# rampasek/GraphGPS

Hardware: NVIDIA H100
Metric: graphs/sec GPSLayer fwd+bwd (higher is better)
Workload: dtype f32

## Files before the change

graphgps_b200/_lib.py:

```python
from __future__ import annotations

import ctypes as C
import os

import torch

_HERE = os.path.dirname(os.path.abspath(__file__))
LIB_PATH = os.path.join(_HERE, "libgps_b200.so")

GPS_OK, GPS_ERR_ARG, GPS_ERR_UNSUPPORTED, GPS_ERR_CUDA = 0, -1, -2, -3
LOCAL = {"None": 0, "CustomGatedGCN": 1, "GINE": 2, "GCN": 3}
GLOBAL = {"None": 0, "Transformer": 1, "Performer": 2}
ACT = {"relu": 0, "gelu": 1}
PRECISION = {"fp32": 0, "bf16": 1}
NORM = {"batch": 0, "none": 1}

_fp = C.c_void_p


class GpsGraph(C.Structure):
    _fields_ = [("N", C.c_int64), ("E", C.c_int64), ("B", C.c_int64),
                ("dst_ptr", _fp), ("dst_src", _fp), ("dst_eid", _fp),
                ("src_ptr", _fp), ("src_dst", _fp), ("src_eid", _fp), ("graph_ptr", _fp)]

# ... 23 lines not shown
        ("x", _fp), ("edge_attr", _fp), ("x_out", _fp), ("edge_out", _fp),
        ("gcn_A", GpsLinear), ("gcn_B", GpsLinear), ("gcn_C", GpsLinear), ("gcn_D", GpsLinear),
        ("gcn_E", GpsLinear),
        ("bn_node_x", GpsBatchNorm), ("bn_edge_e", GpsBatchNorm),
        ("gine_lin0", GpsLinear), ("gine_lin1", GpsLinear),
        ("attn_in", GpsLinear), ("attn_out", GpsLinear),
        ("perf_q", GpsLinear), ("perf_k", GpsLinear), ("perf_v", GpsLinear),
        ("perf_proj", _fp), ("perf_features", C.c_int64), ("perf_dim_head", C.c_int64),
        ("norm1_local", GpsBatchNorm), ("norm1_attn", GpsBatchNorm), ("norm2", GpsBatchNorm),
        ("ff1", GpsLinear), ("ff2", GpsLinear),
        ("grad_x_out", _fp), ("grad_edge_out", _fp), ("grad_x", _fp), ("grad_edge_attr", _fp),
        ("saved", _fp), ("saved_bytes", C.c_int64),
        ("workspace", _fp), ("workspace_bytes", C.c_int64),
        ("offset_dev", _fp),
        ("gcn_conv", GpsLinear),
        ("ev_grads_early", _fp),
        ("x_planes_in", GpsPlanes), ("e_planes_in", GpsPlanes), ("x_planes_out", GpsPlanes), ("e_planes_out", GpsPlanes),
        ("wplanes", _fp), ("wplanes_bytes", C.c_int64), ("wplanes_valid", C.c_int32), ("reserved2", C.c_int32),
        ("ev_grads_mid", _fp), ("ev_grads_done", _fp),
        ("pe", _fp), ("pe_dim", C.c_int64), ("grad_pe", _fp), ("pe_mlp0", GpsLinear), ("pe_mlp1", GpsLinear),
    ]


class GpsLayerPlan(C.Structure):
    _fields_ = [("saved_bytes", C.c_int64), ("fwd_workspace_bytes", C.c_int64),
                ("bwd_workspace_bytes", C.c_int64), ("fwd_launches", C.c_int64),
                ("bwd_launches", C.c_int64), ("wplanes_bytes", C.c_int64)]


_i64, _i32, _f32, _u64 = C.c_int64, C.c_int32, C.c_float, C.c_uint64
SYMBOLS = {
    "gps_last_error": (C.c_char_p, []),
    "gps_abi_version": (C.c_int, []),
    "gps_build_arch": (C.c_char_p, []),
    "gps_graph_bytes": (_i64, [_i64, _i64, _i64]),
    "gps_graph_build": (C.c_int, [_fp, _fp, _i64, _i64, _i64, _fp, _i64, C.POINTER(GpsGraph), _fp]),
    "gps_layer_plan": (C.c_int, [C.POINTER(GpsLayerArgs), C.POINTER(GpsLayerPlan)]),
    "gps_layer_forward": (C.c_int, [C.POINTER(GpsLayerArgs), _fp]),
    "gps_layer_backward": (C.c_int, [C.POINTER(GpsLayerArgs), _fp]),
    "gps_linear_forward": (C.c_int, [_fp, _i64, _fp, _i64, _fp, _fp, _i64, _i64, _i64, _i64, _i32, _i32, _fp]),
    "gps_gemm": (C.c_int, [_fp, _i64, _i32, _fp, _i64, _i32, _fp, _i64, _i64, _i64, _i64, _i32, _i32, _i32, _fp]),
    "gps_gatedgcn_aggregate_forward": (C.c_int, [C.POINTER(GpsGraph), _i64, _fp, _fp, _fp, _fp, _i64, _fp, _fp,
                                                 _fp, _fp, _fp]),
    "gps_gine_aggregate_forward": (C.c_int, [C.POINTER(GpsGraph), _i64, _fp, _fp, _f32, _fp, _fp]),
    "gps_gatedgcn_aggregate_forward_gated": (C.c_int, [C.POINTER(GpsGraph), _i64, _fp, _fp, _fp, _fp, _i64, _fp, _fp,
                                                       _fp, _fp, _fp, _fp]),
    "gps_gatedgcn_aggregate_backward": (C.c_int, [C.POINTER(GpsGraph), _i64, _fp, _fp, _i64, _fp, _fp, _i64, _fp, _fp,
                                                  _fp, C.POINTER(GpsPlanes), C.POINTER(GpsPlanes), _fp]),
    "gps_eslap_forward": (C.c_int, [C.POINTER(GpsGraph), _fp, _i64, _i64, _i32, _fp, _fp, _fp, _fp, _fp, _fp, _fp]),
    "gps_eslap_workspace_bytes": (_i64, [_i64, _i64]),
    "gps_eslap_backward": (C.c_int, [C.POINTER(GpsGraph), _fp, _i64, _i64, _i32, _fp, _fp, _fp, _i64, _fp, _fp, _fp,
                                     _fp, _fp, _fp, _fp, _i64, _fp, _fp, _fp, _fp, _fp, _i32, _fp]),
    "gps_gine_aggregate_backward": (C.c_int, [C.POINTER(GpsGraph), _i64, _fp, _fp, _fp, _f32, _fp, _fp, _fp, _fp]),
    "gps_gcn_aggregate_forward": (C.c_int, [C.POINTER(GpsGraph), _i64, _fp, _i64, _fp, _fp, _fp, _fp, _f32, _u64, _u64,
                                            _fp, _fp]),
    "gps_gcn_aggregate_backward": (C.c_int, [C.POINTER(GpsGraph), _i64, _fp, _fp, _fp, _i64, C.POINTER(GpsPlanes), _fp]),
    "gps_attention_forward": (C.c_int, [C.POINTER(GpsGraph), _i64, _i64, _fp, _fp, _fp, _i64, _fp, _i64, _fp,
                                        _f32, _u64, _u64, _fp]),
    "gps_attention_backward": (C.c_int, [C.POINTER(GpsGraph), _i64, _i64, _fp, _fp, _fp, _i64, _fp, _fp, _i64,
                                         _fp, _fp, _fp, _fp, _fp, _i64, _f32, _u64, _u64, _fp]),
    "gps_attention_forward_tc": (C.c_int, [C.POINTER(GpsGraph), _i64, _i64, _fp, _fp, _i64, _fp, _i64, _fp, _f32, _u64, _u64,
                                           _i32, _fp]),
    "gps_dropout_mask": (C.c_int, [_fp, _i64, _i64, _f32, _u64, _u64, _i32, _fp]),
    "gps_to_planes": (C.c_int, [_fp, _i64, _i64, _i64, _fp, _fp, _i64, _fp]),
    "gps_gemm_planes": (C.c_int, [_fp, _fp, _i64, _i32, _fp, _fp, _i64, _i32, _fp, _i64, _fp, _fp, _i64, _i64, _i64, _i64,
                                  _i32, _i32, _fp, _fp]),
    "gps_fallback_count": (C.c_ulonglong, []),
    "gps_launch_count": (C.c_ulonglong, []),
    "gps_debug_set": (None, [C.c_int]),
    "gps_debug_tma": (None, [C.c_int, _fp]),
    "gps_debug_attn": (None, [_fp]),
}

_lib = None


def load():
    global _lib
    if _lib is not None:
        return _lib
    if not os.path.exists(LIB_PATH):
        raise RuntimeError(
            f"{LIB_PATH} not found: build it with `python -m graphgps_b200.build` "
            "(nvcc, sm_90a). graphgps_b200 has no CPU/eager fallback.")
    lib = C.CDLL(LIB_PATH)
    for name, (res, args) in SYMBOLS.items():
        fn = getattr(lib, name)
        fn.restype = res
        fn.argtypes = args
    if lib.gps_abi_version() != 3:
        raise RuntimeError("libgps_b200.so ABI version mismatch")
    _lib = lib
    return lib
# ... 20 lines not shown
```

graphgps_b200/csrc/gemm.cuh:

```cuda
#pragma once
#include <cuda.h>

#include "common.cuh"

namespace gps {

struct GemmParams {
  int M = 0, N = 0, K = 0;
  const float* A = nullptr; int lda = 0; int ta = 0;
  const float* B = nullptr; int ldb = 0; int tb = 0;
  float* C = nullptr; int ldc = 0;
  const float* bias = nullptr;
  float* C_pre = nullptr; int ldpre = 0;
  int act = -1;
  const float* mask_src = nullptr; int ldmask = 0; int mask_act = -1;
  int mask_is_post = 0;
  float p_drop = 0.f; uint64_t seed = 0, offset = 0; int site = 0;
  const unsigned long long* offset_dev = nullptr;
  float p_drop2 = 0.f; int site2 = 0;
  const float* R1 = nullptr; int ldr1 = 0;
  const float* R2 = nullptr; int ldr2 = 0;
  double* stats = nullptr;
  int splitk = 1;
  float* colsum_a = nullptr;
  int precision = GPS_PREC_FP32;
  Planes Ap, Bp, Cp;
  int cp_hd = 0, cp_hd_pad = 0, cp_col0 = 0;
  struct BnRed { const float* z = nullptr; int ldz = 0; const float* mean = nullptr; const float* invstd = nullptr; double* sums = nullptr; };
  BnRed bnred[2];
};

struct ToPlanesItem { const float* src; int64_t ld; int rows; int cols; Planes dst; };
int to_planes(const ToPlanesItem* items, int n, cudaStream_t stream);
int gemm_tma(const GemmParams& p, cudaStream_t stream);
int make_tensor_map(const __nv_bfloat16* hi, const __nv_bfloat16* lo, int planes, int64_t rows, int64_t cols, int64_t ld,
                    int box_rows, CUtensorMap* out);
void gemm_tma_set_force_bn(int bn);
void gemm_tma_set_trace(unsigned long long* buf);

int gemm_simt(const GemmParams& p, cudaStream_t stream);
int gemm_tc(const GemmParams& p, cudaStream_t stream);
void gemm_tc_set_debug(int v);
int gemm(const GemmParams& p, cudaStream_t stream);

}
```

graphgps_b200/csrc/gemm_tma.cu:

```cuda
#include <cooperative_groups.h>
#include <cuda.h>
#include <cuda_bf16.h>

#include <mutex>
#include <unordered_map>

#include "gemm.cuh"
#include "tc_ptx.cuh"

namespace gps {

namespace {

using namespace tc;
namespace cgrp = cooperative_groups;

constexpr int BM = 128;
constexpr int BK = 64;
constexpr int kEpiWarps = 8;
constexpr int kTmaWarp = 8;
constexpr int kThreads = 288;
constexpr int kATile = BM * BK * 2;
constexpr int kBlock = 64 * BK * 2;
constexpr int kMaxSplits = 8;

struct TmaArgs {
  GemmParams p;
  int BN, nb_blocks, stages, kb_per_split, planes;
  int debug;
  unsigned long long* trace;
};

__device__ __forceinline__ unsigned long long gtimer() {
  unsigned long long t;
  asm volatile("mov.u64 %0, %globaltimer;" : "=l"(t));
  return t;
}
#define GPS_TRACE(slot)                                                                         \
  do {                                                                                          \
    if (a.trace && cta_lin < 256) a.trace[cta_lin * 16 + (slot)] = gtimer();                    \
  } while (0)

template <bool A_MN, bool B_MN, int BN_T, bool SPLIT>
__global__ void __launch_bounds__(kThreads, BN_T == 64 ? 2 : 1)
k_gemm_tma(const __grid_constant__ CUtensorMap tmA, const __grid_constant__ CUtensorMap tmB, const TmaArgs a) {
  extern __shared__ __align__(1024) uint8_t smem_raw[];
  const GemmParams& p = a.p;
  uint8_t* smem = reinterpret_cast<uint8_t*>((reinterpret_cast<uintptr_t>(smem_raw) + 1023) & ~(uintptr_t)1023);
  const int planes = a.planes;
  const int b_tile = B_MN ? a.nb_blocks * kBlock : BN_T * 128;
  const int stage_bytes = planes * (kATile + b_tile);
  const int S = a.stages;
  uint64_t* bars = reinterpret_cast<uint64_t*>(smem + (size_t)S * stage_bytes);
  float* red = reinterpret_cast<float*>(bars + 2 * S + 2);
  float* ctot = red + 16 * 16 * 8;
  const int nsplit = (int)gridDim.z;

  const int tid = threadIdx.x, warp = tid >> 5, lane = tid & 31;
  const int m0 = blockIdx.y * BM, n0 = blockIdx.x * a.BN;
  const int nkb_total = (p.K + BK - 1) / BK;
  const int kb_begin = blockIdx.z * a.kb_per_split;
  const int kb_end = min(nkb_total, kb_begin + a.kb_per_split);
  const int nkb = kb_end - kb_begin;
  const bool do_colsum = A_MN && p.colsum_a != nullptr && blockIdx.x == 0;
  const int cta_lin = (blockIdx.z * gridDim.y + blockIdx.y) * gridDim.x + blockIdx.x;

  if (tid == 0) {
    GPS_TRACE(0);
    if (a.trace && cta_lin < 256) {
      unsigned smid;
      asm volatile("mov.u32 %0, %smid;" : "=r"(smid));
      a.trace[cta_lin * 16 + 8] = smid;
    }
    for (int s = 0; s < S; ++s) {
      mbar_init(smem_u32(&bars[s]), 1);
      mbar_init(smem_u32(&bars[S + s]), kEpiWarps);
    }
    fence_barrier_init();
  }
  if (warp == kTmaWarp && lane == 0) {
    tma_prefetch_desc(&tmA);
    tma_prefetch_desc(&tmB);
  }
  __syncthreads();
  if (tid == 0) GPS_TRACE(1);

  if (warp == kTmaWarp) {
// ... 9 lines not shown
        const uint32_t full = smem_u32(&bars[s]);
        mbar_arrive_expect_tx(full, tx);
        const int k0 = (kb_begin + i) * BK;
        const uint32_t sa = smem_u32(smem + (size_t)s * stage_bytes);
        const uint32_t sb = sa + planes * kATile;
        for (int pl = 0; pl < planes; ++pl) {
          if (!A_MN) {
            tma_tile_3d(sa + pl * kATile, &tmA, k0, m0, pl, full);
          } else {
            for (int b = 0; b < a_blocks; ++b) tma_tile_3d(sa + pl * kATile + b * kBlock, &tmA, m0 + 64 * b, k0, pl, full);
          }
          if (!B_MN) {
            tma_tile_3d(sb + pl * b_tile, &tmB, k0, n0, pl, full);
          } else {
            for (int b = 0; b < b_blocks; ++b) tma_tile_3d(sb + pl * b_tile + b * kBlock, &tmB, n0 + 64 * b, k0, pl, full);
          }
        }
        if (i == 0) GPS_TRACE(2);
      }
      GPS_TRACE(9);
    }
    __syncwarp();
    if (nsplit > 1) {
      cgrp::this_cluster().sync();
      cgrp::this_cluster().sync();
    }
  } else {
    const int wg = warp >> 2;
    float acc[BN_T / 2];
#pragma unroll
    for (int e = 0; e < BN_T / 2; ++e) acc[e] = 0.f;
    float csum[8];
#pragma unroll
    for (int e = 0; e < 8; ++e) csum[e] = 0.f;
    const int cm = tid & 15, kq = tid >> 4;
    constexpr uint32_t a_lbo = A_MN ? kBlock : 16, b_lbo = B_MN ? kBlock : 16;
    constexpr uint32_t a_kstep = A_MN ? 2048 : 32, b_kstep = B_MN ? 2048 : 32;
    for (int i = 0; i < nkb; ++i) {
      const int s = i % S;
      if (lane == 0) mbar_wait(smem_u32(&bars[s]), (uint32_t)(i / S) & 1u);
      __syncwarp();
      if (i == 0 && tid == 0) GPS_TRACE(3);
      if (i == nkb - 1 && tid == 0) GPS_TRACE(10);
      const uint8_t* st = smem + (size_t)s * stage_bytes;
      const uint32_t sa_hi = smem_u32(st) + (uint32_t)wg * 8192u;
      const uint32_t sb_hi = smem_u32(st) + planes * kATile;
      const uint32_t sa_lo = sa_hi + kATile;
      const uint32_t sb_lo = sb_hi + b_tile;
// ... 70 lines not shown
      cgrp::cluster_group cluster = cgrp::this_cluster();
      cluster.sync();
      const int c4n = a.BN >> 2;
      for (int idx = tid; idx < (hi - lo) * c4n; idx += kEpiWarps * 32) {
        const int r = lo + idx / c4n, c = (idx % c4n) * 4;
        float4 sum = f4zero();
        for (int k = 0; k < nsplit; ++k)
          sum = f4add(sum, *reinterpret_cast<const float4*>(cluster.map_shared_rank(stage, k) + r * sld + c));
        *reinterpret_cast<float4*>(stage + r * sld + c) = sum;
      }
      if (do_colsum && blockIdx.z == 0 && tid < 128 && m0 + tid < p.M) {
        float tot = 0.f;
        for (int k = 0; k < nsplit; ++k) tot += cluster.map_shared_rank(ctot, k)[tid];
        atomicAdd(&p.colsum_a[m0 + tid], tot);
      }
      cluster.sync();
    }
    const int G = a.BN >> 2;
    const int rpp = kEpiWarps * 32 / G;
    const int rip = tid / G, cg = tid - rip * G;
    const int col = n0 + cg * 4;
    const bool col_ok = rip < rpp && col < p.N;
    const int rows_here = min(BM, p.M - m0);
    const bool colstats = p.stats || p.bnred[0].sums || p.bnred[1].sums;
    if (col_ok) {
      const int nrows = rip < rows_here ? (rows_here - rip + rpp - 1) / rpp : 0;
      const int64_t row0 = m0 + rip;
      float* sp = stage + rip * sld + cg * 4;
      const int s_st = rpp * sld;
      float* cp = p.C ? p.C + row0 * p.ldc + col : nullptr;
      const int64_t c_st = (int64_t)rpp * p.ldc;
      const float* r1 = p.R1 ? p.R1 + row0 * p.ldr1 + col : nullptr;
      const int64_t r1_st = (int64_t)rpp * p.ldr1;
      const float* r2 = p.R2 ? p.R2 + row0 * p.ldr2 + col : nullptr;
      const int64_t r2_st = (int64_t)rpp * p.ldr2;
      if (p.splitk > 1) {
        for (int r = lo + rip; r < min(hi, rows_here); r += rpp) {
          const int64_t row = m0 + r;
          float4 w = *reinterpret_cast<const float4*>(stage + r * sld + cg * 4);
          if (p.R1) w = f4add(w, ld4(p.R1 + row * p.ldr1 + col));
          if (p.R2) w = f4add(w, ld4(p.R2 + row * p.ldr2 + col));
          atomicAdd(reinterpret_cast<float4*>(p.C + row * p.ldc + col), w);
        }
      } else {
        const bool fast = !p.C_pre && !(p.mask_src && !p.mask_is_post) && p.p_drop == 0.f && p.p_drop2 == 0.f &&
                          (p.act < 0 || p.act == GPS_ACT_RELU);
        const float4 bb = p.bias ? ld4(p.bias + col) : f4zero();
        const float* mk = p.mask_src ? p.mask_src + row0 * p.ldmask + col : nullptr;
        const int64_t mk_st = (int64_t)rpp * p.ldmask;
        int pcol = col, npad = 0;
        if (p.cp_hd > 0) {
          const int cl = col - (p.cp_col0), hq = cl / p.cp_hd, cw = cl - hq * p.cp_hd;
          pcol = hq * p.cp_hd_pad + cw;
          npad = (cw + 4 == p.cp_hd) ? p.cp_hd_pad - p.cp_hd : 0;
        }
        __nv_bfloat16* ph = p.Cp.hi ? p.Cp.hi + row0 * p.Cp.ld + pcol : nullptr;
        __nv_bfloat16* pl = p.Cp.lo ? p.Cp.lo + row0 * p.Cp.ld + pcol : nullptr;
        const int64_t p_st = (int64_t)rpp * p.Cp.ld;
        const bool relu = p.act == GPS_ACT_RELU;
        if (fast) {
// ... 67 lines not shown
            if (r1) w = f4add(w, ld4(r1 + k * r1_st));
            if (r2) w = f4add(w, ld4(r2 + k * r2_st));
            if (cp) st4(cp + k * c_st, w);
            if (ph) {
              planes_store4(p.Cp, row, pcol, w);
              for (int z = 0; z < npad; z += 4) planes_store4(p.Cp, row, pcol + 4 + z, f4zero());
            }
            if (colstats) *reinterpret_cast<float4*>(sp + k * s_st) = w;
          }
        }
      }
    }
    if (colstats) {
      asm volatile("bar.sync 1, 256;" ::: "memory");
      for (int t = tid; t < 16 * G; t += kEpiWarps * 32) {
        const int y = t / G, g = t - y * G, c = n0 + g * 4;
        if (c >= p.N) continue;
        const GemmParams::BnRed& b0 = p.bnred[0];
        const GemmParams::BnRed& b1 = p.bnred[1];
        float4 bm0 = f4zero(), bi0 = f4zero(), bm1 = f4zero(), bi1 = f4zero();
        if (b0.sums) { bm0 = f4scale(ld4(b0.mean + c), -1.f); bi0 = ld4(b0.invstd + c); }
        if (b1.sums) { bm1 = f4scale(ld4(b1.mean + c), -1.f); bi1 = ld4(b1.invstd + c); }
        float4 s1 = f4zero(), s2 = f4zero(), q0 = f4zero(), q1 = f4zero();
        for (int r = y; r < rows_here; r += 16) {
          const float4 w = *reinterpret_cast<const float4*>(stage + r * sld + g * 4);
          const int64_t row = m0 + r;
          s1 = f4add(s1, w);
          s2 = f4fma(w, w, s2);
          if (b0.sums) q0 = f4fma(w, f4mul(f4add(ld4(b0.z + row * b0.ldz + c), bm0), bi0), q0);
          if (b1.sums) q1 = f4fma(w, f4mul(f4add(ld4(b1.z + row * b1.ldz + c), bm1), bi1), q1);
        }
        float* o = stage + y * sld + g * 4;
        *reinterpret_cast<float4*>(o) = s1;
        *reinterpret_cast<float4*>(o + 16 * sld) = s2;
        *reinterpret_cast<float4*>(o + 32 * sld) = q0;
        *reinterpret_cast<float4*>(o + 48 * sld) = q1;
      }
      asm volatile("bar.sync 1, 256;" ::: "memory");
      if (tid < G && n0 + tid * 4 < p.N) {
        float4 t[4] = {f4zero(), f4zero(), f4zero(), f4zero()};
        for (int y = 0; y < 16; ++y)
#pragma unroll
          for (int k = 0; k < 4; ++k) t[k] = f4add(t[k], *reinterpret_cast<const float4*>(stage + (y + 16 * k) * sld + tid * 4));
        const int c0 = n0 + tid * 4;
        auto add4 = [&](double* dst, float4 v) {
          atomic_add_f64(dst + 0, (double)v.x); atomic_add_f64(dst + 1, (double)v.y);
          atomic_add_f64(dst + 2, (double)v.z); atomic_add_f64(dst + 3, (double)v.w);
        };
        if (p.stats) {
          add4(p.stats + c0, t[0]);
          add4(p.stats + (int64_t)p.N + c0, t[1]);
        }
        if (p.bnred[0].sums) {
          add4(p.bnred[0].sums + c0, t[0]);
          add4(p.bnred[0].sums + (int64_t)p.N + c0, t[2]);
        }
        if (p.bnred[1].sums) {
          add4(p.bnred[1].sums + c0, t[0]);
          add4(p.bnred[1].sums + (int64_t)p.N + c0, t[3]);
        }
      }
    }
  }

  if (tid == 0) GPS_TRACE(6);
  if (a.trace) {
// ... 95 lines not shown
    cudaLaunchConfig_t cfg = {};
    cfg.gridDim = grid;
    cfg.blockDim = dim3(kThreads);
    cfg.dynamicSmemBytes = smem;
    cfg.stream = stream;
    cudaLaunchAttribute attr[1];
    attr[0].id = cudaLaunchAttributeClusterDimension;
    attr[0].val.clusterDim.x = 1;
    attr[0].val.clusterDim.y = 1;
    attr[0].val.clusterDim.z = grid.z;
    cfg.attrs = attr;
    cfg.numAttrs = 1;
    GPS_CUDA(cudaLaunchKernelEx(&cfg, k_gemm_tma<A_MN, B_MN, BN_T, SPLIT>, tA, tB, a));
  }
  GPS_LAUNCH_CHECK();
  return GPS_OK;
}
template <bool A_MN, bool B_MN, int BN_T>
int launch(const CUtensorMap& tA, const CUtensorMap& tB, const TmaArgs& a, dim3 grid, size_t smem, cudaStream_t stream) {
  return a.planes == 2 ? launch1<A_MN, B_MN, BN_T, true>(tA, tB, a, grid, smem, stream)
                       : launch1<A_MN, B_MN, BN_T, false>(tA, tB, a, grid, smem, stream);
}

int g_tma_force_bn = 0;
unsigned long long* g_tma_trace = nullptr;
int g_tma_debug = 0;

}

void gemm_tma_set_force_bn(int bn) { g_tma_force_bn = bn & 0xFFFF; g_tma_debug = bn >> 16; }
void gemm_tma_set_trace(unsigned long long* buf) { g_tma_trace = buf; }

int gemm_tma(const GemmParams& p, cudaStream_t stream) {
  if (p.M <= 0 || p.N <= 0) return GPS_OK;
  if (p.K <= 0 || !p.Ap.hi || !p.Bp.hi) return GPS_ERR_UNSUPPORTED;
  const bool split = p.precision == GPS_PREC_FP32;
  const int planes = split ? 2 : 1;
  if (split && (!p.Ap.lo || !p.Bp.lo)) return GPS_ERR_UNSUPPORTED;
  if (!aligned16(p.Ap.hi) || !aligned16(p.Bp.hi) || p.Ap.ld % 8 || p.Bp.ld % 8 || p.N % 4) return GPS_ERR_UNSUPPORTED;
  if (split && (!aligned16(p.Ap.lo) || !aligned16(p.Bp.lo))) return GPS_ERR_UNSUPPORTED;
  if ((p.C && (!aligned16(p.C) || p.ldc % 4)) || (!p.C && !p.Cp.hi)) return GPS_ERR_UNSUPPORTED;
  if (p.Cp.hi && (p.Cp.ld % 4 || (reinterpret_cast<uintptr_t>(p.Cp.hi) & 7) || (p.Cp.lo && (reinterpret_cast<uintptr_t>(p.Cp.lo) & 7))))
    return GPS_ERR_UNSUPPORTED;
  if ((p.bias && !aligned16(p.bias)) || (p.R1 && (!aligned16(p.R1) || p.ldr1 % 4)) ||
      (p.R2 && (!aligned16(p.R2) || p.ldr2 % 4)) || (p.mask_src && (!aligned16(p.mask_src) || p.ldmask % 4)) ||
      (p.C_pre && (!aligned16(p.C_pre) || p.ldpre % 4)))
    return GPS_ERR_UNSUPPORTED;
  if (p.splitk > 1 && (p.bias || p.act >= 0 || p.mask_src || p.stats || p.C_pre || p.p_drop != 0.f || p.p_drop2 != 0.f ||
                       p.Cp.hi || !p.C)) {
    set_error("gemm: split-K supports the plain fp32 product (+ residuals) only");
    return GPS_ERR_ARG;
  }
  if (p.colsum_a && !p.ta) {
    set_error("gemm: colsum_a needs ta == 1");
    return GPS_ERR_ARG;
  }
  if ((p.bnred[0].sums || p.bnred[1].sums) &&
      (p.splitk > 1 || p.C_pre || (p.mask_src && !p.mask_is_post) || p.p_drop != 0.f || p.p_drop2 != 0.f ||
       (p.act >= 0 && p.act != GPS_ACT_RELU))) {
    set_error("gemm: fused BatchNorm-backward reductions need the plain epilogue (no split-K / dropout / GELU)");
    return GPS_ERR_ARG;
  }
  const int mt = (int)ceil_div(p.M, BM);
  const int nkb = (int)ceil_div(p.K, BK);
  const int splits_hint = p.splitk > 1 ? min(kMaxSplits, min(p.splitk, nkb)) : 1;
  const auto width_ok = [&](int bn) {
    return bn == 64 || bn == 128 || (bn == 152 && !p.tb) || (bn == 256 && !p.ta);
  };
  int bestBN = 0;
  long bestCost = 0;
  for (const int bn : {64, 128, 152, 256}) {
    if (!width_ok(bn)) continue;
    const long tiles = (long)mt * ceil_div(p.N, bn) * splits_hint;
    const long cost = bn != 64 ? ceil_div(tiles, (long)kNumSMs) * bn : tiles <= kNumSMs ? 64 : ceil_div(tiles, 2L * kNumSMs) * 160;
    if (!bestBN || cost <= bestCost) { bestCost = cost; bestBN = bn; }
  }
  if (g_tma_force_bn) {
    if (!width_ok(g_tma_force_bn)) return GPS_ERR_UNSUPPORTED;
    bestBN = g_tma_force_bn;
  }
  TmaArgs a;
  a.p = p;
  a.BN = bestBN;
  a.nb_blocks = a.BN / 64;
  a.planes = planes;
  const bool narrow = a.nb_blocks == 1;
  const int stage_bytes = planes * (kATile + (p.tb ? a.nb_blocks * kBlock : a.BN * 128));
  const int fixed = 1024  + 1024  + 16 * 16 * 8 * 4 + 128 * 4;
  int stages = ((narrow ? 112 : 226) * 1024 - fixed) / stage_bytes;
  if (stages > 8) stages = 8;
  if (stages < 2) return GPS_ERR_UNSUPPORTED;
  GPS_REQUIRE((size_t)stages * stage_bytes >= (size_t)BM * (a.BN + 4) * 4, GPS_ERR_ARG,
              "gemm_tma: BN %d: the staging tile does not fit the operand stages", a.BN);
  a.stages = stages;
  int splitk = p.splitk > 1 ? p.splitk : 1;
  if (splitk > kMaxSplits) splitk = kMaxSplits;
  if (splitk > nkb) splitk = nkb;
  a.kb_per_split = (int)ceil_div(nkb, splitk);
  splitk = (int)ceil_div(nkb, a.kb_per_split);
  a.p.splitk = p.splitk > 1 ? 2 : 1;
  a.trace = g_tma_trace;
  a.debug = g_tma_debug;
  const bool amn = p.ta != 0, bmn = p.tb != 0;
  CUtensorMap tA, tB;
  GPS_TRY(tensor_map(p.Ap.hi, p.Ap.lo, planes, amn ? p.K : p.M, amn ? p.M : p.K, p.Ap.ld, amn ? 64 : BM, &tA));
  GPS_TRY(tensor_map(p.Bp.hi, p.Bp.lo, planes, bmn ? p.K : p.N, bmn ? p.N : p.K, p.Bp.ld, bmn ? 64 : a.BN, &tB));
  const size_t smem = (size_t)stages * stage_bytes + fixed;
  dim3 grid((unsigned)ceil_div(p.N, a.BN), (unsigned)mt, (unsigned)splitk);
#define GPS_TMA_CASE(AM, BMN)                                                                              \
  if (amn == AM && bmn == BMN) {                                                                           \
    if (a.BN == 64) return launch<AM, BMN, 64>(tA, tB, a, grid, smem, stream);                            \
    if (a.BN == 128) return launch<AM, BMN, 128>(tA, tB, a, grid, smem, stream);                          \
  }
  GPS_TMA_CASE(false, false)
  GPS_TMA_CASE(false, true)
  GPS_TMA_CASE(true, false)
  GPS_TMA_CASE(true, true)
#undef GPS_TMA_CASE
  if (a.BN == 152 && !bmn)
    return amn ? launch<true, false, 152>(tA, tB, a, grid, smem, stream) : launch<false, false, 152>(tA, tB, a, grid, smem, stream);
  if (a.BN == 256 && !amn)
    return bmn ? launch<false, true, 256>(tA, tB, a, grid, smem, stream) : launch<false, false, 256>(tA, tB, a, grid, smem, stream);
  return GPS_ERR_UNSUPPORTED;
}

namespace {
struct ToPlanesDesc {
  ToPlanesItem it[16];
  int start[17];
  int n;
};
// ... 53 lines not shown
```

graphgps_b200/csrc/layer.cu:

```cuda
#include <stdarg.h>
#include <string.h>

#include <algorithm>
#include <atomic>

#include "gemm.cuh"
#include "kernels.cuh"

namespace gps {

int perf_supported(int64_t dim_head, int64_t features);
int64_t perf_mp();
int perf_prep(const float* P, int64_t m, float* Pn, const GpsGraph& g, int64_t H, int* nmax, float* gmax, int* argk,
              cudaStream_t st);
int perf_features_fwd(float* fq, float* fk, const float* Q, const float* K, const GpsGraph& g, int64_t H, int64_t m,
                      float* gmax, int* argq, int* argk, cudaStream_t st);
int perf_linattn_fwd(const GpsGraph& g, int64_t H, int64_t m, const int* nmax, const float* qf, const float* kf,
                     const float* V, const float* gmax, float* O, cudaStream_t st);
int perf_linattn_bwd(const GpsGraph& g, int64_t H, int64_t m, const int* nmax, const float* qf, const float* kf,
                     const float* V, const float* gmax, const float* gO, float* g_qf, float* g_kf, float* gV,
                     float* ggmax, cudaStream_t st);
int perf_features_bwd(float* g_fq, float* g_fk, const float* fq, const float* fk, const float* Q, const float* K,
                      float* gQ, float* gK, const GpsGraph& g, int64_t H, int64_t m, const int* argq, const int* argk,
                      float* ggmax, cudaStream_t st);
// ... 839 lines not shown
  const int64_t N = P.N, E = P.E, d = P.d;
  const int act = a->act;
  DropCfg nodrop;
  auto sums = [&](int which) { return P.bsums + (int64_t)which * 2 * d; };
  GPS_CUDA(cudaMemsetAsync(P.bsums, 0, (size_t)P.nbn * 2 * d * sizeof(double), st));
  Side* sd;
  GPS_TRY(side_stream(&sd));
  cudaStream_t s2 = sd->s;
  auto wfork = [&](cudaStream_t from) -> int { return sd->order(from, s2); };
  const bool two_branches = (P.gated || P.gine || P.gcn) && (P.attn || P.perf);
  cudaStream_t sa = two_branches ? sd->s3 : st;
  cudaStream_t se = sd->s4;
  const int opt = opt_flags();
  auto record_ev = [&](void* ev, cudaStream_t s) -> int {
    if (!ev) return GPS_OK;
    cudaStreamCaptureStatus cs = cudaStreamCaptureStatusNone;
    GPS_CUDA(cudaStreamIsCapturing(s, &cs));
    GPS_CUDA(cudaEventRecordWithFlags((cudaEvent_t)ev, s, cs == cudaStreamCaptureStatusActive ? cudaEventRecordExternal
                                                                                               : cudaEventRecordDefault));
    return GPS_OK;
  };
  auto early_done = [&]() -> int { return record_ev(a->ev_grads_early, s2); };
  auto mid_done = [&]() -> int { return record_ev(a->ev_grads_mid, s2); };
  const bool gx_splitk = P.Wy >= 1024 && N > 0;
  if (P.Wy) {
    GPS_TRY(wfork(st));
    GPS_CUDA(cudaMemsetAsync(P.gWcat, 0, (size_t)(P.Wy * d + P.Wy) * sizeof(float), s2));
  }
  if (gx_splitk) GPS_CUDA(cudaMemsetAsync(a->grad_x, 0, (size_t)(N * d) * sizeof(float), st));

  if (P.gated) {
    GPS_TRY(sd->order(st, se));
    BnView ve = bn_view(P, BN_E, a->bn_edge_e);
    if (a->grad_edge_out && E > 0) {
      GPS_TRY(bn_bwd_reduce(a->grad_edge_out, d, P.ehat, d, E, d, ve, act, P.drop(GPS_SITE_GCN_E), sums(BN_E), se));
      GPS_TRY(bn_bwd_apply(a->grad_edge_out, d, P.ehat, d, E, d, ve, act, P.drop(GPS_SITE_GCN_E), sums(BN_E), P.g_e, d,
                           a->bn_edge_e.grad_weight, a->bn_edge_e.grad_bias, se, P.grads_accumulate));
    } else {
      if (E > 0) GPS_CUDA(cudaMemsetAsync(P.g_e, 0, (size_t)(E * d) * sizeof(float), se));
      if (a->bn_edge_e.grad_weight && !P.grads_prezeroed)
        GPS_CUDA(cudaMemsetAsync(a->bn_edge_e.grad_weight, 0, d * sizeof(float), se));
      if (a->bn_edge_e.grad_bias && !P.grads_prezeroed)
        GPS_CUDA(cudaMemsetAsync(a->bn_edge_e.grad_bias, 0, d * sizeof(float), se));
    }
  }

  const float* g_t = P.nonorm ? a->grad_x_out : P.g_t;
  if (!P.nonorm) {
    BnView v2 = bn_view(P, BN_2, a->norm2);
    GPS_TRY(bn_bwd_reduce(a->grad_x_out, d, P.t, d, N, d, v2, -1, nodrop, sums(BN_2), st));
    GPS_TRY(bn_bwd_apply(a->grad_x_out, d, P.t, d, N, d, v2, -1, nodrop, sums(BN_2), P.g_t, d, a->norm2.grad_weight,
                         a->norm2.grad_bias, st, P.grads_accumulate, P.gt_p));
// ... 169 lines not shown
    GPS_TRY(dropmul(P, {g_xloc, d}, P.g_tmp3, Planes(), GPS_SITE_LOCAL, st, &g_h));
    if (a->gcn_conv.grad_bias) {
      if (!P.grads_prezeroed) GPS_CUDA(cudaMemsetAsync(a->gcn_conv.grad_bias, 0, (size_t)d * sizeof(float), st));
      GPS_TRY(colsum(g_h.f, d, N, d, a->gcn_conv.grad_bias, st));
    }
    GPS_TRY(gcn_bwd(a->graph, d, g_h.f, P.dinv, P.gY1, P.Wy, st, P.gY1_p));
    GPS_TRY(wfork(st));
    GPS_TRY(mid_done());
    g_x_local = g_xloc;
  }

  if (two_branches) GPS_TRY(sd->order(sa, st));

  if (P.Wy) {
    const Operand gY1{P.gY1, P.Wy, P.gY1_p};
    GPS_TRY(wfork(st));
    GPS_TRY(wgrad_add(P, gY1, {a->x, d, P.x_p}, N, P.Wy, d, P.gWcat, P.gbcat, s2));
    PackDesc pdsc = pack_desc(P);
    k_unpack<<<(unsigned)P.Wy, 128, 0, s2>>>(pdsc, P.gWcat, P.gbcat, P.grads_accumulate ? 1 : 0);
    GPS_LAUNCH_CHECK();
    GemmParams g = linear_dgrad(P, N, d, P.Wy, gY1, {P.Wcat, d, P.Wcat_p}, a->grad_x, d);
    g.R1 = g_x_local; g.ldr1 = (int)d;
    g.R2 = P.attn ? g_hA : (P.perf ? P.g_xp : nullptr); g.ldr2 = (int)d;
    if (gx_splitk) g.splitk = 4;
    GPS_TRY(gemm(g, st));
  } else if (g_x_local) {
    GPS_TRY(add3(g_x_local, d, P.perf ? P.g_xp : nullptr, d, nullptr, 0, a->grad_x, d, N, d, st));
  } else {
    GPS_TRY(add3(P.g_xp, d, nullptr, 0, nullptr, 0, a->grad_x, d, N, d, st));
  }
  GPS_TRY(sd->join(st));
  GPS_TRY(record_ev(a->ev_grads_done, st));
  return GPS_OK;
}

}

using namespace gps;

extern "C" const char* gps_last_error(void) { return g_err; }
extern "C" int gps_abi_version(void) { return GPS_ABI_VERSION; }
extern "C" const char* gps_build_arch(void) { return "sm_90a"; }
extern "C" unsigned long long gps_launch_count(void) { return g_launches.load(); }
extern "C" unsigned long long gps_fallback_count(void) { return g_fallbacks.load(); }

extern "C" int gps_to_planes(const float* src, int64_t ld, int64_t rows, int64_t cols, void* hi, void* lo, int64_t ldp,
                             void* stream) {
  GPS_REQUIRE(src && hi, GPS_ERR_ARG, "gps_to_planes: null argument");
  ToPlanesItem it{src, ld, (int)rows, (int)cols, Planes{(__nv_bfloat16*)hi, (__nv_bfloat16*)lo, ldp}};
  return to_planes(&it, 1, (cudaStream_t)stream);
}

extern "C" int gps_gemm_planes(const void* A_hi, const void* A_lo, int64_t lda, int32_t ta, const void* B_hi,
                               const void* B_lo, int64_t ldb, int32_t tb, float* C, int64_t ldc, void* C_hi, void* C_lo,
                               int64_t ldcp, int64_t M, int64_t N, int64_t K, int32_t splitk, int32_t precision,
                               float* colsum_a, void* stream) {
  GemmParams g;
  g.M = (int)M; g.N = (int)N; g.K = (int)K;
  g.ta = ta; g.tb = tb; g.C = C; g.ldc = (int)ldc;
  g.Ap = Planes{(__nv_bfloat16*)A_hi, (__nv_bfloat16*)A_lo, lda};
  g.Bp = Planes{(__nv_bfloat16*)B_hi, (__nv_bfloat16*)B_lo, ldb};
  g.Cp = Planes{(__nv_bfloat16*)C_hi, (__nv_bfloat16*)C_lo, ldcp};
  g.splitk = splitk < 1 ? 1 : splitk; g.precision = precision; g.colsum_a = colsum_a;
  int rc = gemm_tma(g, (cudaStream_t)stream);
  if (rc == GPS_ERR_UNSUPPORTED) set_error("gps_gemm_planes: the TMA kernel does not take this shape/alignment");
  return rc;
}
extern "C" void gps_debug_set(int v) { gemm_tc_set_debug(v); }
extern "C" void gps_debug_tma(int force_bn, void* trace) {
  gemm_tma_set_force_bn(force_bn);
  gemm_tma_set_trace((unsigned long long*)trace);
}
extern "C" void gps_debug_attn(void* buf) { attention_tc_set_debug((float*)buf); }

extern "C" int gps_layer_plan(const GpsLayerArgs* args, GpsLayerPlan* plan) {
  GPS_REQUIRE(args && plan, GPS_ERR_ARG, "gps_layer_plan: null argument");
  Plan P;
  GPS_TRY(make_plan(args, &P, false));
  plan->saved_bytes = P.saved_bytes;
  plan->fwd_workspace_bytes = P.fwd_bytes;
  plan->bwd_workspace_bytes = P.bwd_bytes;
  plan->fwd_launches = 0;
  plan->bwd_launches = 0;
  plan->wplanes_bytes = P.wplanes_bytes;
  return GPS_OK;
}

extern "C" int gps_layer_forward(const GpsLayerArgs* args, void* stream) {
  GPS_REQUIRE(args, GPS_ERR_ARG, "gps_layer_forward: null args");
  return layer_forward(args, (cudaStream_t)stream);
}
// ... 186 lines not shown
```

include/gps_b200.h:

```cpp
#ifndef GPS_B200_H_
#define GPS_B200_H_

#include <stdint.h>

#ifdef __cplusplus
extern "C" {
#endif

#define GPS_ABI_VERSION 3

enum { GPS_OK = 0, GPS_ERR_ARG = -1, GPS_ERR_UNSUPPORTED = -2, GPS_ERR_CUDA = -3 };

enum { GPS_LOCAL_NONE = 0, GPS_LOCAL_GATEDGCN = 1, GPS_LOCAL_GINE = 2, GPS_LOCAL_GCN = 3 };
enum { GPS_GLOBAL_NONE = 0, GPS_GLOBAL_TRANSFORMER = 1, GPS_GLOBAL_PERFORMER = 2 };
enum { GPS_ACT_RELU = 0, GPS_ACT_GELU = 1 };
enum { GPS_PREC_FP32 = 0, GPS_PREC_BF16 = 1 };
enum { GPS_NORM_BATCH = 0, GPS_NORM_NONE = 1 };

const char* gps_last_error(void);
int gps_abi_version(void);
const char* gps_build_arch(void);
unsigned long long gps_launch_count(void);
void gps_debug_set(int v);
void gps_debug_tma(int force_bn, void* trace);
void gps_debug_attn(void* buf);

typedef struct {
  int64_t N, E, B;
  const int32_t* dst_ptr;
  const int32_t* dst_src;
  const int32_t* dst_eid;
  const int32_t* src_ptr;
  const int32_t* src_dst;
  const int32_t* src_eid;
  const int32_t* graph_ptr;
} GpsGraph;

int64_t gps_graph_bytes(int64_t N, int64_t E, int64_t B);
int gps_graph_build(const int64_t* edge_index, const int64_t* batch, int64_t N, int64_t E,
                    int64_t B, void* storage, int64_t storage_bytes, GpsGraph* out,
                    void* stream);

typedef struct {
  const float* weight;
  const float* bias;
  float* running_mean;
  float* running_var;
// ... 123 lines not shown
int gps_gcn_aggregate_forward(const GpsGraph* g, int64_t d, const float* Y, int64_t ldy, const float* bias,
                              const float* x, float* dinv, float* xloc, float p_drop, uint64_t seed, uint64_t offset,
                              double* stats, void* stream);
int gps_gcn_aggregate_backward(const GpsGraph* g, int64_t d, const float* g_h, const float* dinv, float* gY,
                               int64_t ldg, const GpsPlanes* gY_planes, void* stream);

int gps_attention_forward(const GpsGraph* g, int64_t heads, int64_t hd, const float* Q,
                          const float* K, const float* V, int64_t ld, float* O, int64_t ldo,
                          float* lse, float p_drop, uint64_t seed, uint64_t offset, void* stream);
int gps_attention_forward_tc(const GpsGraph* g, int64_t heads, int64_t hd, const void* qkv_hi, const void* qkv_lo,
                             int64_t ld, float* O, int64_t ldo, float* lse, float p_drop, uint64_t seed,
                             uint64_t offset, int32_t precision, void* stream);
int gps_attention_backward(const GpsGraph* g, int64_t heads, int64_t hd, const float* Q,
                           const float* K, const float* V, int64_t ld, const float* O,
                           const float* dO, int64_t ldo, const float* lse, float* delta,
                           float* dQ, float* dK, float* dV, int64_t ldg, float p_drop,
                           uint64_t seed, uint64_t offset, void* stream);

int gps_to_planes(const float* src, int64_t ld, int64_t rows, int64_t cols, void* hi, void* lo, int64_t ldp,
                  void* stream);
int gps_gemm_planes(const void* A_hi, const void* A_lo, int64_t lda, int32_t ta, const void* B_hi, const void* B_lo,
                    int64_t ldb, int32_t tb, float* C, int64_t ldc, void* C_hi, void* C_lo, int64_t ldcp, int64_t M,
                    int64_t N, int64_t K, int32_t splitk, int32_t precision, float* colsum_a, void* stream);
unsigned long long gps_fallback_count(void);

int gps_dropout_mask(float* mask, int64_t rows, int64_t cols, float p, uint64_t seed,
                     uint64_t offset, int32_t site, void* stream);

#ifdef __cplusplus
}
#endif
#endif
```

Baseline: 339,200.

## Let the TMA GEMM tile policy choose split-K and cluster-reduce column stats

The TMA GEMM launcher now searches split-K factors (up to 4) jointly with tile width, using a cost model of waves times K-blocks plus a fixed split overhead. This lets small-M, large-K GEMMs fill more SMs without callers asking for split-K. The fused column-statistics epilogue now reduces partial sums across the split-K cluster through distributed shared memory, with extra cluster syncs in the producer warp. The hardcoded split-K=4 and grad_x memset on the dgrad path are removed. A debug hook for the last launch shape and an epilogue-capable planes GEMM entry point are also added.

After: 345,300 (median of 6 runs). +1.8%, better.

```diff
diff --git a/graphgps_b200/_lib.py b/graphgps_b200/_lib.py
--- a/graphgps_b200/_lib.py
+++ b/graphgps_b200/_lib.py
@@ -69,6 +69,16 @@
     ]
 
 
+class GpsGemmEpilogue(C.Structure):
+    _fields_ = [("bias", _fp), ("C_pre", _fp), ("ldpre", C.c_int64), ("act", C.c_int32), ("mask_act", C.c_int32),
+                ("mask", _fp), ("ldmask", C.c_int64), ("mask_is_post", C.c_int32),
+                ("p_drop", C.c_float), ("site", C.c_int32), ("p_drop2", C.c_float), ("site2", C.c_int32),
+                ("seed", C.c_uint64), ("offset", C.c_uint64),
+                ("R1", _fp), ("ldr1", C.c_int64), ("R2", _fp), ("ldr2", C.c_int64),
+                ("stats", _fp), ("cp_hd", C.c_int32), ("cp_hd_pad", C.c_int32),
+                ("bn_z", _fp), ("bn_ldz", C.c_int64), ("bn_mean", _fp), ("bn_invstd", _fp), ("bn_sums", _fp)]
+
+
 class GpsLayerPlan(C.Structure):
     _fields_ = [("saved_bytes", C.c_int64), ("fwd_workspace_bytes", C.c_int64),
                 ("bwd_workspace_bytes", C.c_int64), ("fwd_launches", C.c_int64),
@@ -112,10 +122,13 @@
     "gps_to_planes": (C.c_int, [_fp, _i64, _i64, _i64, _fp, _fp, _i64, _fp]),
     "gps_gemm_planes": (C.c_int, [_fp, _fp, _i64, _i32, _fp, _fp, _i64, _i32, _fp, _i64, _fp, _fp, _i64, _i64, _i64, _i64,
                                   _i32, _i32, _fp, _fp]),
+    "gps_gemm_planes_epilogue": (C.c_int, [_fp, _fp, _i64, _i32, _fp, _fp, _i64, _i32, _fp, _i64, _fp, _fp, _i64, _i64,
+                                           _i64, _i64, _i32, C.POINTER(GpsGemmEpilogue), _fp]),
     "gps_fallback_count": (C.c_ulonglong, []),
     "gps_launch_count": (C.c_ulonglong, []),
     "gps_debug_set": (None, [C.c_int]),
     "gps_debug_tma": (None, [C.c_int, _fp]),
+    "gps_debug_tma_last": (None, [_fp]),
     "gps_debug_attn": (None, [_fp]),
 }
 
diff --git a/graphgps_b200/csrc/gemm.cuh b/graphgps_b200/csrc/gemm.cuh
--- a/graphgps_b200/csrc/gemm.cuh
+++ b/graphgps_b200/csrc/gemm.cuh
@@ -36,6 +36,7 @@
 int make_tensor_map(const __nv_bfloat16* hi, const __nv_bfloat16* lo, int planes, int64_t rows, int64_t cols, int64_t ld,
                     int box_rows, CUtensorMap* out);
 void gemm_tma_set_force_bn(int bn);
+void gemm_tma_last_launch(int* out);
 void gemm_tma_set_trace(unsigned long long* buf);
 
 int gemm_simt(const GemmParams& p, cudaStream_t stream);
diff --git a/graphgps_b200/csrc/gemm_tma.cu b/graphgps_b200/csrc/gemm_tma.cu
--- a/graphgps_b200/csrc/gemm_tma.cu
+++ b/graphgps_b200/csrc/gemm_tma.cu
@@ -23,6 +23,8 @@
 constexpr int kATile = BM * BK * 2;
 constexpr int kBlock = 64 * BK * 2;
 constexpr int kMaxSplits = 8;
+constexpr int kMaxPolicySplits = 4;
+constexpr long kSplitKb16 = 56;
 
 struct TmaArgs {
   GemmParams p;
@@ -63,6 +65,7 @@
   const int kb_end = min(nkb_total, kb_begin + a.kb_per_split);
   const int nkb = kb_end - kb_begin;
   const bool do_colsum = A_MN && p.colsum_a != nullptr && blockIdx.x == 0;
+  const bool colstats = p.stats || p.bnred[0].sums || p.bnred[1].sums;
   const int cta_lin = (blockIdx.z * gridDim.y + blockIdx.y) * gridDim.x + blockIdx.x;
 
   if (tid == 0) {
@@ -118,8 +121,7 @@
     }
     __syncwarp();
     if (nsplit > 1) {
-      cgrp::this_cluster().sync();
-      cgrp::this_cluster().sync();
+      for (int b = 0; b < (colstats ? 4 : 2); ++b) cgrp::this_cluster().sync();
     }
   } else {
     const int wg = warp >> 2;
@@ -236,11 +238,12 @@
     const int col = n0 + cg * 4;
     const bool col_ok = rip < rpp && col < p.N;
     const int rows_here = min(BM, p.M - m0);
-    const bool colstats = p.stats || p.bnred[0].sums || p.bnred[1].sums;
+    const int row_end = min(hi, rows_here);
     if (col_ok) {
-      const int nrows = rip < rows_here ? (rows_here - rip + rpp - 1) / rpp : 0;
-      const int64_t row0 = m0 + rip;
-      float* sp = stage + rip * sld + cg * 4;
+      const int r_first = lo + rip;
+      const int nrows = r_first < row_end ? (row_end - r_first + rpp - 1) / rpp : 0;
+      const int64_t row0 = m0 + r_first;
+      float* sp = stage + r_first * sld + cg * 4;
       const int s_st = rpp * sld;
       float* cp = p.C ? p.C + row0 * p.ldc + col : nullptr;
       const int64_t c_st = (int64_t)rpp * p.ldc;
@@ -249,7 +252,7 @@
       const float* r2 = p.R2 ? p.R2 + row0 * p.ldr2 + col : nullptr;
       const int64_t r2_st = (int64_t)rpp * p.ldr2;
       if (p.splitk > 1) {
-        for (int r = lo + rip; r < min(hi, rows_here); r += rpp) {
+        for (int r = r_first; r < row_end; r += rpp) {
           const int64_t row = m0 + r;
           float4 w = *reinterpret_cast<const float4*>(stage + r * sld + cg * 4);
           if (p.R1) w = f4add(w, ld4(p.R1 + row * p.ldr1 + col));
@@ -363,7 +366,7 @@
         if (b0.sums) { bm0 = f4scale(ld4(b0.mean + c), -1.f); bi0 = ld4(b0.invstd + c); }
         if (b1.sums) { bm1 = f4scale(ld4(b1.mean + c), -1.f); bi1 = ld4(b1.invstd + c); }
         float4 s1 = f4zero(), s2 = f4zero(), q0 = f4zero(), q1 = f4zero();
-        for (int r = y; r < rows_here; r += 16) {
+        for (int r = lo + ((y - lo) & 15); r < row_end; r += 16) {
           const float4 w = *reinterpret_cast<const float4*>(stage + r * sld + g * 4);
           const int64_t row = m0 + r;
           s1 = f4add(s1, w);
@@ -378,11 +381,32 @@
         *reinterpret_cast<float4*>(o + 48 * sld) = q1;
       }
       asm volatile("bar.sync 1, 256;" ::: "memory");
-      if (tid < G && n0 + tid * 4 < p.N) {
-        float4 t[4] = {f4zero(), f4zero(), f4zero(), f4zero()};
+      const bool own_col = tid < G && n0 + tid * 4 < p.N;
+      float4 t[4] = {f4zero(), f4zero(), f4zero(), f4zero()};
+      if (own_col) {
         for (int y = 0; y < 16; ++y)
 #pragma unroll
           for (int k = 0; k < 4; ++k) t[k] = f4add(t[k], *reinterpret_cast<const float4*>(stage + (y + 16 * k) * sld + tid * 4));
+      }
+      if (nsplit > 1) {
+        if (own_col) {
+#pragma unroll
+          for (int k = 0; k < 4; ++k) *reinterpret_cast<float4*>(stage + 16 * k * sld + tid * 4) = t[k];
+        }
+        cgrp::cluster_group cluster = cgrp::this_cluster();
+        cluster.sync();
+        if (own_col && blockIdx.z == 0) {
+#pragma unroll
+          for (int k = 0; k < 4; ++k) t[k] = f4zero();
+          for (int q = 0; q < nsplit; ++q) {
+            const float* o = cluster.map_shared_rank(stage, q) + tid * 4;
+#pragma unroll
+            for (int k = 0; k < 4; ++k) t[k] = f4add(t[k], *reinterpret_cast<const float4*>(o + 16 * k * sld));
+          }
+        }
+        cluster.sync();
+      }
+      if (own_col && blockIdx.z == 0) {
         const int c0 = n0 + tid * 4;
         auto add4 = [&](double* dst, float4 v) {
           atomic_add_f64(dst + 0, (double)v.x); atomic_add_f64(dst + 1, (double)v.y);
@@ -524,14 +548,16 @@
                        : launch1<A_MN, B_MN, BN_T, false>(tA, tB, a, grid, smem, stream);
 }
 
-int g_tma_force_bn = 0;
+int g_tma_force = 0;
 unsigned long long* g_tma_trace = nullptr;
 int g_tma_debug = 0;
-
-}
-
-void gemm_tma_set_force_bn(int bn) { g_tma_force_bn = bn & 0xFFFF; g_tma_debug = bn >> 16; }
+int g_tma_last[3] = {0, 0, 0};
+
+}
+
+void gemm_tma_set_force_bn(int bn) { g_tma_force = bn & 0xFFFF; g_tma_debug = bn >> 16; }
 void gemm_tma_set_trace(unsigned long long* buf) { g_tma_trace = buf; }
+void gemm_tma_last_launch(int* out) { for (int i = 0; i < 3; ++i) out[i] = g_tma_last[i]; }
 
 int gemm_tma(const GemmParams& p, cudaStream_t stream) {
   if (p.M <= 0 || p.N <= 0) return GPS_OK;
@@ -557,30 +583,54 @@
     set_error("gemm: colsum_a needs ta == 1");
     return GPS_ERR_ARG;
   }
-  if ((p.bnred[0].sums || p.bnred[1].sums) &&
-      (p.splitk > 1 || p.C_pre || (p.mask_src && !p.mask_is_post) || p.p_drop != 0.f || p.p_drop2 != 0.f ||
-       (p.act >= 0 && p.act != GPS_ACT_RELU))) {
+  const bool bnred = p.bnred[0].sums || p.bnred[1].sums;
+  if (bnred && (p.splitk > 1 || p.C_pre || (p.mask_src && !p.mask_is_post) || p.p_drop != 0.f || p.p_drop2 != 0.f ||
+                (p.act >= 0 && p.act != GPS_ACT_RELU))) {
     set_error("gemm: fused BatchNorm-backward reductions need the plain epilogue (no split-K / dropout / GELU)");
     return GPS_ERR_ARG;
   }
+  const int force_bn = g_tma_force & 0xFFF, force_splits = (g_tma_force >> 12) & 0xF;
+  if (bnred && force_splits > 1) {
+    set_error("gemm: fused BatchNorm-backward reductions do not run with split-K");
+    return GPS_ERR_ARG;
+  }
   const int mt = (int)ceil_div(p.M, BM);
   const int nkb = (int)ceil_div(p.K, BK);
-  const int splits_hint = p.splitk > 1 ? min(kMaxSplits, min(p.splitk, nkb)) : 1;
   const auto width_ok = [&](int bn) {
     return bn == 64 || bn == 128 || (bn == 152 && !p.tb) || (bn == 256 && !p.ta);
   };
-  int bestBN = 0;
+  if (force_bn && !width_ok(force_bn)) return GPS_ERR_UNSUPPORTED;
+  const auto width_cost = [&](int bn, int s) {
+    const long tiles = (long)mt * ceil_div(p.N, bn) * s;
+    const bool lone_ok = p.splitk > 1 || ceil_div(nkb, s) <= 4;
+    return bn != 64 ? ceil_div(tiles, (long)kNumSMs) * bn
+                    : tiles <= kNumSMs && lone_ok ? 64 : ceil_div(tiles, 2L * kNumSMs) * 160;
+  };
+  const int splits_hint = p.splitk > 1 ? min(kMaxSplits, min(p.splitk, nkb)) : 1;
+  const int s_max = p.splitk > 1 ? splits_hint : bnred ? 1 : min(kMaxPolicySplits, nkb);
+  int bestBN = 0, bestS = 0;
   long bestCost = 0;
-  for (const int bn : {64, 128, 152, 256}) {
-    if (!width_ok(bn)) continue;
-    const long tiles = (long)mt * ceil_div(p.N, bn) * splits_hint;
-    const long cost = bn != 64 ? ceil_div(tiles, (long)kNumSMs) * bn : tiles <= kNumSMs ? 64 : ceil_div(tiles, 2L * kNumSMs) * 160;
-    if (!bestBN || cost <= bestCost) { bestCost = cost; bestBN = bn; }
-  }
-  if (g_tma_force_bn) {
-    if (!width_ok(g_tma_force_bn)) return GPS_ERR_UNSUPPORTED;
-    bestBN = g_tma_force_bn;
-  }
+  for (int s = splits_hint; s <= s_max; ++s) {
+    const int kbps = (int)ceil_div(nkb, s);
+    if (p.splitk <= 1 && ceil_div(nkb, kbps) != s) continue;
+    for (const int bn : {64, 128, 152, 256}) {
+      if (!width_ok(bn)) continue;
+      if (p.splitk <= 1 && s > 1 && (long)mt * ceil_div(p.N, bn) * s > (bn == 64 ? 2L : 1L) * kNumSMs) continue;
+      const long cost = width_cost(bn, s) * (16L * kbps + (s > 1 ? kSplitKb16 : 0));
+      if (!bestBN || cost < bestCost || (cost == bestCost && s == bestS)) { bestCost = cost; bestBN = bn; bestS = s; }
+    }
+  }
+  if (force_splits) {
+    bestS = min(force_splits, min(kMaxSplits, nkb));
+    bestS = (int)ceil_div(nkb, ceil_div(nkb, bestS));
+    bestBN = 0;
+    for (const int bn : {64, 128, 152, 256}) {
+      if (!width_ok(bn)) continue;
+      const long cost = width_cost(bn, bestS);
+      if (!bestBN || cost <= bestCost) { bestCost = cost; bestBN = bn; }
+    }
+  }
+  if (force_bn) bestBN = force_bn;
   TmaArgs a;
   a.p = p;
   a.BN = bestBN;
@@ -595,11 +645,8 @@
   GPS_REQUIRE((size_t)stages * stage_bytes >= (size_t)BM * (a.BN + 4) * 4, GPS_ERR_ARG,
               "gemm_tma: BN %d: the staging tile does not fit the operand stages", a.BN);
   a.stages = stages;
-  int splitk = p.splitk > 1 ? p.splitk : 1;
-  if (splitk > kMaxSplits) splitk = kMaxSplits;
-  if (splitk > nkb) splitk = nkb;
-  a.kb_per_split = (int)ceil_div(nkb, splitk);
-  splitk = (int)ceil_div(nkb, a.kb_per_split);
+  a.kb_per_split = (int)ceil_div(nkb, bestS);
+  const int splitk = (int)ceil_div(nkb, a.kb_per_split);
   a.p.splitk = p.splitk > 1 ? 2 : 1;
   a.trace = g_tma_trace;
   a.debug = g_tma_debug;
@@ -609,6 +656,7 @@
   GPS_TRY(tensor_map(p.Bp.hi, p.Bp.lo, planes, bmn ? p.K : p.N, bmn ? p.N : p.K, p.Bp.ld, bmn ? 64 : a.BN, &tB));
   const size_t smem = (size_t)stages * stage_bytes + fixed;
   dim3 grid((unsigned)ceil_div(p.N, a.BN), (unsigned)mt, (unsigned)splitk);
+  g_tma_last[0] = (int)(grid.x * grid.y * grid.z); g_tma_last[1] = a.BN; g_tma_last[2] = splitk;
 #define GPS_TMA_CASE(AM, BMN)                                                                              \
   if (amn == AM && bmn == BMN) {                                                                           \
     if (a.BN == 64) return launch<AM, BMN, 64>(tA, tB, a, grid, smem, stream);                            \
diff --git a/graphgps_b200/csrc/layer.cu b/graphgps_b200/csrc/layer.cu
--- a/graphgps_b200/csrc/layer.cu
+++ b/graphgps_b200/csrc/layer.cu
@@ -885,12 +885,10 @@
   };
   auto early_done = [&]() -> int { return record_ev(a->ev_grads_early, s2); };
   auto mid_done = [&]() -> int { return record_ev(a->ev_grads_mid, s2); };
-  const bool gx_splitk = P.Wy >= 1024 && N > 0;
   if (P.Wy) {
     GPS_TRY(wfork(st));
     GPS_CUDA(cudaMemsetAsync(P.gWcat, 0, (size_t)(P.Wy * d + P.Wy) * sizeof(float), s2));
   }
-  if (gx_splitk) GPS_CUDA(cudaMemsetAsync(a->grad_x, 0, (size_t)(N * d) * sizeof(float), st));
 
   if (P.gated) {
     GPS_TRY(sd->order(st, se));
@@ -1106,7 +1104,6 @@
     GemmParams g = linear_dgrad(P, N, d, P.Wy, gY1, {P.Wcat, d, P.Wcat_p}, a->grad_x, d);
     g.R1 = g_x_local; g.ldr1 = (int)d;
     g.R2 = P.attn ? g_hA : (P.perf ? P.g_xp : nullptr); g.ldr2 = (int)d;
-    if (gx_splitk) g.splitk = 4;
     GPS_TRY(gemm(g, st));
   } else if (g_x_local) {
     GPS_TRY(add3(g_x_local, d, P.perf ? P.g_xp : nullptr, d, nullptr, 0, a->grad_x, d, N, d, st));
@@ -1150,7 +1147,32 @@
   if (rc == GPS_ERR_UNSUPPORTED) set_error("gps_gemm_planes: the TMA kernel does not take this shape/alignment");
   return rc;
 }
+extern "C" int gps_gemm_planes_epilogue(const void* A_hi, const void* A_lo, int64_t lda, int32_t ta, const void* B_hi,
+                                        const void* B_lo, int64_t ldb, int32_t tb, float* C, int64_t ldc, void* C_hi,
+                                        void* C_lo, int64_t ldcp, int64_t M, int64_t N, int64_t K, int32_t precision,
+                                        const GpsGemmEpilogue* e, void* stream) {
+  GPS_REQUIRE(e, GPS_ERR_ARG, "gps_gemm_planes_epilogue: null epilogue");
+  GemmParams g;
+  g.M = (int)M; g.N = (int)N; g.K = (int)K;
+  g.ta = ta; g.tb = tb; g.C = C; g.ldc = (int)ldc;
+  g.Ap = Planes{(__nv_bfloat16*)A_hi, (__nv_bfloat16*)A_lo, lda};
+  g.Bp = Planes{(__nv_bfloat16*)B_hi, (__nv_bfloat16*)B_lo, ldb};
+  g.Cp = Planes{(__nv_bfloat16*)C_hi, (__nv_bfloat16*)C_lo, ldcp};
+  g.precision = precision;
+  g.bias = e->bias; g.C_pre = e->C_pre; g.ldpre = (int)e->ldpre; g.act = e->act;
+  g.mask_src = e->mask; g.ldmask = (int)e->ldmask; g.mask_act = e->mask_act; g.mask_is_post = e->mask_is_post;
+  g.p_drop = e->p_drop; g.site = e->site; g.p_drop2 = e->p_drop2; g.site2 = e->site2; g.seed = e->seed; g.offset = e->offset;
+  g.R1 = e->R1; g.ldr1 = (int)e->ldr1; g.R2 = e->R2; g.ldr2 = (int)e->ldr2;
+  g.stats = e->stats;
+  g.cp_hd = e->cp_hd; g.cp_hd_pad = e->cp_hd_pad;
+  g.bnred[0].z = e->bn_z; g.bnred[0].ldz = (int)e->bn_ldz; g.bnred[0].mean = e->bn_mean; g.bnred[0].invstd = e->bn_invstd;
+  g.bnred[0].sums = e->bn_sums;
+  int rc = gemm_tma(g, (cudaStream_t)stream);
+  if (rc == GPS_ERR_UNSUPPORTED) set_error("gps_gemm_planes_epilogue: the TMA kernel does not take this shape/alignment");
+  return rc;
+}
 extern "C" void gps_debug_set(int v) { gemm_tc_set_debug(v); }
+extern "C" void gps_debug_tma_last(int32_t* out) { gemm_tma_last_launch(out); }
 extern "C" void gps_debug_tma(int force_bn, void* trace) {
   gemm_tma_set_force_bn(force_bn);
   gemm_tma_set_trace((unsigned long long*)trace);
diff --git a/include/gps_b200.h b/include/gps_b200.h
--- a/include/gps_b200.h
+++ b/include/gps_b200.h
@@ -23,6 +23,7 @@
 unsigned long long gps_launch_count(void);
 void gps_debug_set(int v);
 void gps_debug_tma(int force_bn, void* trace);
+void gps_debug_tma_last(int32_t* out);
 void gps_debug_attn(void* buf);
 
 typedef struct {
@@ -192,6 +193,23 @@
 int gps_gemm_planes(const void* A_hi, const void* A_lo, int64_t lda, int32_t ta, const void* B_hi, const void* B_lo,
                     int64_t ldb, int32_t tb, float* C, int64_t ldc, void* C_hi, void* C_lo, int64_t ldcp, int64_t M,
                     int64_t N, int64_t K, int32_t splitk, int32_t precision, float* colsum_a, void* stream);
+typedef struct {
+  const float* bias;
+  float* C_pre; int64_t ldpre;
+  int32_t act; int32_t mask_act;
+  const float* mask; int64_t ldmask; int32_t mask_is_post;
+  float p_drop; int32_t site; float p_drop2; int32_t site2;
+  uint64_t seed, offset;
+  const float* R1; int64_t ldr1;
+  const float* R2; int64_t ldr2;
+  double* stats;
+  int32_t cp_hd, cp_hd_pad;
+  const float* bn_z; int64_t bn_ldz; const float* bn_mean; const float* bn_invstd; double* bn_sums;
+} GpsGemmEpilogue;
+int gps_gemm_planes_epilogue(const void* A_hi, const void* A_lo, int64_t lda, int32_t ta, const void* B_hi,
+                             const void* B_lo, int64_t ldb, int32_t tb, float* C, int64_t ldc, void* C_hi, void* C_lo,
+                             int64_t ldcp, int64_t M, int64_t N, int64_t K, int32_t precision,
+                             const GpsGemmEpilogue* epi, void* stream);
 unsigned long long gps_fallback_count(void);
 
 int gps_dropout_mask(float* mask, int64_t rows, int64_t cols, float p, uint64_t seed,
```
